# chymaera96/GraFP

Hardware: AMD Instinct MI355X
Metric: clips/sec contrastive step @ batch 1024 (higher is better)
Workload: dtype bf16; 1 GPU; contrastive step at global batch 1024 (1024 pairs/GPU x 1 GPU, global negatives), 1 s clips @16 kHz, mel->kNN-graph->GNN->NT-Xent, fwd+bwd+Adam, random-init GraphEncoder-t (18.4M params); global_batch=1024, parallelism=dp1, k=3

## Files before the change

grafp_amd/csrc/knn_split.hip:

```cpp
#include "dma_ring.h"
#include "elemio.h"
#include "knngraph.h"
#include "tuning.h"

namespace grafp {

constexpr int KS_KC = 32;
constexpr int KS_PLANE = KS_KC * KNN_TR * 2;
constexpr int KS_STAGE = 4 * KS_PLANE;
constexpr int KS_LDS = 2 * KS_STAGE + 3 * KNN_TR * 4;
constexpr float KS_SHIFT = 9.765625e-4f;

template <typename T>
__global__ __launch_bounds__(256) void knn_normalize_split_kernel(const T *__restrict__ x, int64_t sb, int64_t sc,
                                                                  float *__restrict__ den_out, float *__restrict__ sq,
                                                                  unsigned short *__restrict__ xh,
                                                                  unsigned short *__restrict__ xl, int C, int N,
                                                                  int *__restrict__ counters) {
    const int n = blockIdx.x * 256 + threadIdx.x;
    const int b = blockIdx.y;
    if (blockIdx.x == 0 && b == 0 && threadIdx.x < 2) counters[threadIdx.x] = 0;
    if (n >= N) return;
    const T *xb = x + (size_t)b * sb + n;
    const size_t o = (size_t)b * C * N + n;
// ... 110 lines not shown
        const int blk = t / nch, ch = t - blk * nch;
        const unsigned short *s = src0 + (size_t)(ch * KS_KC) * N + (wave >= 2 ? 0 : blk * KNN_TR);
        const unsigned st = lds0 + (t & 1) * KS_STAGE + wave * KS_PLANE;
#pragma unroll
        for (int i = 0; i < 8; ++i) gm_dma16(s + (size_t)(4 * i) * N, st + i * 1024);
        if (ch == 0 && wave < 2)
            gm_dma4(sqb + blk * KNN_TR + wave * 64 + lane, lds0 + 2 * KS_STAGE + ((blk % 3) * KNN_TR + wave * 64) * 4);
    };

    int foff[4];
#pragma unroll
    for (int tt = 0; tt < 4; ++tt) foff[tt] = ks_frag_offset(tt, lane, half);
    const int qoff = ks_frag_offset(wave, lane, half);

    f32x16 acc[4], prev[4];
#pragma unroll
    for (int t = 0; t < 4; ++t)
#pragma unroll
        for (int r = 0; r < 16; ++r) { acc[t][r] = 0.0f; prev[t][r] = 0.0f; }
    KeyList<K + 1> best;
    best.init();

    auto insert = [&](const f32x16 (&a)[4], int e, int sq_base, unsigned lane_bits) {
        const int loc_c = (e >> 4) * 32 + ((e & 15) & 3) + 8 * ((e & 15) >> 2);
        const float d = __builtin_fmaf(-2.0f, a[e >> 4][e & 15], dq) + sSq[sq_base + loc_c + 4 * half];
        best.push((__float_as_uint(d) & key_mask) | lane_bits | (unsigned)loc_c);
    };

    dma_chunk(0);
    gm_wait_vm<0>();
    __syncthreads();
    for (int blk = 0; blk < nblk; ++blk) {
        const int sq_prev = ((blk + 2) % 3) * KNN_TR;
        const unsigned bits_prev = (unsigned)((blk - 1) * KNN_TR) | (unsigned)(4 * half);
        for (int ch = 0; ch < nch; ++ch) {
            const int t = blk * nch + ch;
            if (t + 1 < T) dma_chunk(t + 1);
            const unsigned char *st = smem + (t & 1) * KS_STAGE;
#pragma unroll
            for (int ks = 0; ks < 2; ++ks) {
                const gm_bf16x8 qh = ks_frag(st + 2 * KS_PLANE, qoff + ks * 16 * 256);
                const gm_bf16x8 ql = ks_frag(st + 3 * KS_PLANE, qoff + ks * 16 * 256);
#pragma unroll
                for (int tt = 0; tt < 4; ++tt) {
                    const gm_bf16x8 ah = ks_frag(st, foff[tt] + ks * 16 * 256);
                    const gm_bf16x8 al = ks_frag(st + KS_PLANE, foff[tt] + ks * 16 * 256);
                    acc[tt] = __builtin_amdgcn_mfma_f32_32x32x16_bf16(al, qh, acc[tt], 0, 0, 0);
                    acc[tt] = __builtin_amdgcn_mfma_f32_32x32x16_bf16(ah, ql, acc[tt], 0, 0, 0);
                    acc[tt] = __builtin_amdgcn_mfma_f32_32x32x16_bf16(ah, qh, acc[tt], 0, 0, 0);
                }
                if (ch == 0 && blk > 0) {
#pragma unroll
                    for (int e = 0; e < 32; ++e) insert(prev, ks * 32 + e, sq_prev, bits_prev);
                }
            }
            gm_wait_vm<0>();
            __syncthreads();
        }
#pragma unroll
        for (int tt = 0; tt < 4; ++tt) {
            prev[tt] = acc[tt];
#pragma unroll
            for (int r = 0; r < 16; ++r) acc[tt][r] = 0.0f;
        }
    }
    {
        const unsigned bits_last = (unsigned)((nblk - 1) * KNN_TR) | (unsigned)(4 * half);
#pragma unroll
        for (int e = 0; e < 64; ++e) insert(prev, e, ((nblk + 2) % 3) * KNN_TR, bits_last);
    }
    unsigned ok[K + 1], onext = (unsigned)__shfl_xor((int)best.next, 32);
#pragma unroll
    for (int t = 0; t <= K; ++t) ok[t] = (unsigned)__shfl_xor((int)best.k[t], 32);
#pragma unroll
    for (int t = 0; t <= K; ++t) best.push(ok[t]);
    best.next = onext < best.next ? onext : best.next;
    if (half == 0)
        ks_classify_store<K>(best, key_mask, margin2, false, (size_t)b * N + myq, idx, unc_count, unc_flag, extra);
}

constexpr int KR_NS = 4;
constexpr int KR_STAGE = 2 * KS_PLANE;
constexpr int KR_NT = 8;
constexpr int KR_LDS = KR_NS * KR_STAGE + KR_NT * KNN_TR * 8;
constexpr float KR_TINY = 1.8189894e-12f;

template <int VE>
__global__ __launch_bounds__(256) void knn_norms_kernel(const unsigned short *__restrict__ x, int64_t sb, int64_t sc,
                                                        float *__restrict__ den_out, float *__restrict__ sq,
                                                        float2 *__restrict__ cs, int B, int C, int N,
                                                        int *__restrict__ counters) {
    const int per = N / VE;
    const int64_t gid = (int64_t)blockIdx.x * 256 + threadIdx.x;
    if (gid < 2) counters[gid] = 0;
    if (gid >= (int64_t)B * per) return;
    const int b = (int)(gid / per), n0 = (int)(gid - (int64_t)b * per) * VE;
    const unsigned short *xb = x + (size_t)b * sb + n0;
    float ss[VE], den[VE], q[VE];
#pragma unroll
    for (int u = 0; u < VE; ++u) ss[u] = 0.0f;
    auto load = [&](int c, unsigned (&w)[VE / 2]) {
        if (VE == 8) {
            const uint4 t = *reinterpret_cast<const uint4 *>(xb + (size_t)c * sc);
            w[0] = t.x; w[1 % (VE / 2)] = t.y; w[2 % (VE / 2)] = t.z; w[3 % (VE / 2)] = t.w;
        } else if (VE == 4) {
            const uint2 t = *reinterpret_cast<const uint2 *>(xb + (size_t)c * sc);
            w[0] = t.x; w[1 % (VE / 2)] = t.y;
        } else {
            w[0] = *reinterpret_cast<const unsigned *>(xb + (size_t)c * sc);
        }
    };
    for (int c = 0; c < C; c += 8) {
        unsigned w[8][VE / 2];
#pragma unroll
        for (int j = 0; j < 8; ++j) load(c + j, w[j]);
#pragma unroll
        for (int j = 0; j < 8; ++j)
#pragma unroll
            for (int e = 0; e < VE / 2; ++e) {
                const float lo = bf16_lo(w[j][e]), hi = bf16_hi(w[j][e]);
                ss[2 * e] = __builtin_fmaf(lo, lo, ss[2 * e]);
                ss[2 * e + 1] = __builtin_fmaf(hi, hi, ss[2 * e + 1]);
            }
    }
#pragma unroll
    for (int u = 0; u < VE; ++u) {
        den[u] = fmaxf(sqrtf(ss[u]), 1e-12f);
        q[u] = 0.0f;
    }
    for (int c = 0; c < C; c += 8) {
        unsigned w[8][VE / 2];
#pragma unroll
        for (int j = 0; j < 8; ++j) load(c + j, w[j]);
#pragma unroll
        for (int j = 0; j < 8; ++j)
#pragma unroll
            for (int e = 0; e < VE / 2; ++e) {
                const float lo = __fdiv_rn(bf16_lo(w[j][e]), den[2 * e]);
                const float hi = __fdiv_rn(bf16_hi(w[j][e]), den[2 * e + 1]);
                q[2 * e] = __builtin_fmaf(lo, lo, q[2 * e]);
                q[2 * e + 1] = __builtin_fmaf(hi, hi, q[2 * e + 1]);
            }
    }
    const size_t o = (size_t)b * N + n0;
#pragma unroll
    for (int u = 0; u < VE; ++u) {
        sq[o + u] = q[u];
        den_out[o + u] = den[u];
    }
    f32x4 *cs4 = reinterpret_cast<f32x4 *>(cs) + (o >> 1);
#pragma unroll
    for (int u = 0; u < VE; u += 2)
        cs4[u >> 1] = f32x4{-2.0f * __frcp_rn(den[u]), -2.0f * __frcp_rn(den[u + 1]), q[u], q[u + 1]};
}

template <int K, typename I>
__global__ __launch_bounds__(256, 2) void knn_topk_raw_kernel(const unsigned short *__restrict__ x, int64_t sb, int64_t sc,
                                                              const float *__restrict__ sq, const float *__restrict__ den,
                                                              const float2 *__restrict__ cs, I *__restrict__ idx,
                                                              int *__restrict__ unc_count,
                                                              unsigned char *__restrict__ unc_flag,
                                                              int *__restrict__ extra,
                                                              int C, int N, int tiles_per_clip, int nblocks,
                                                              float margin2, unsigned key_mask) {
    constexpr int D = KR_NS - 1;
    extern __shared__ __attribute__((aligned(16))) unsigned char smem[];
    const float2 *const sCS = reinterpret_cast<const float2 *>(smem + KR_NS * KR_STAGE);
    const unsigned lds0 = (unsigned)(uintptr_t)(gm_lptr)smem;

    const KnnCoords w = knn_coords(nblocks, tiles_per_clip);
    const int b = w.b, q0 = w.q0, lane = w.lane, half = w.half, l31 = w.l31;
    const int wave = __builtin_amdgcn_readfirstlane(w.wave);
    const int myq = q0 + wave * 32 + l31;
    const float iq = den[(size_t)b * N + myq];
    const float dqi = (sq[(size_t)b * N + myq] + KS_SHIFT) * iq;
    const float2 *csb = cs + (size_t)b * N;

    const int nch = C / KS_KC, nblk = N / KNN_TR, T = nblk * nch;

    const int pl = wave >> 1, hw = wave & 1;
    const int rowl = lane >> 4, sl = lane & 15;
    const int scol = (((sl >> 2) ^ (rowl & 3)) * 4 + (sl & 3)) * 8;
    const unsigned short *src0 = x + (size_t)b * sb + (size_t)(hw * 16 + rowl) * sc + scol + (pl ? q0 : 0);
    auto dma_chunk = [&](int t) {
        const int blk = t / nch, ch = t - blk * nch;
        const unsigned short *s = src0 + (size_t)(ch * KS_KC) * sc + (pl ? 0 : blk * KNN_TR);
        const unsigned st = lds0 + (t % KR_NS) * KR_STAGE + pl * KS_PLANE + hw * 4096;
#pragma unroll
        for (int i = 0; i < 4; ++i) gm_dma16(s + (size_t)(4 * i) * sc, st + i * 1024);
        if (ch == 0 && wave == 0)
            gm_dma16(csb + blk * KNN_TR + lane * 2, lds0 + KR_NS * KR_STAGE + (blk % KR_NT) * (KNN_TR * 8));
    };

    int foff[4];
#pragma unroll
    for (int tt = 0; tt < 4; ++tt) foff[tt] = ks_frag_offset(tt, lane, half);
    const int qoff = ks_frag_offset(wave, lane, half);

    f32x16 acc[4];
    KeyList<K + 1> best;
    best.init();
    bool bad = false;

    const gm_f32x2 iq2 = {iq, iq}, dqi2 = {dqi, dqi};
    unsigned kmv = key_mask;
    asm volatile("" : "+v"(kmv));
    auto insert4 = [&](const f32x16 (&a)[4], int e0, int tb, unsigned lane_bits) {
        const int tt = e0 >> 4, r0 = e0 & 15;
        const int loc_c = tt * 32 + 8 * (r0 >> 2);
        const f32x4 *tp = reinterpret_cast<const f32x4 *>(sCS + tb + loc_c + 4 * half);
        const f32x4 t01 = tp[0], t23 = tp[1];
        const gm_f32x2 d01 = __builtin_elementwise_fma(gm_f32x2{a[tt][r0], a[tt][r0 + 1]}, gm_f32x2{t01[0], t01[1]},
                                                    __builtin_elementwise_fma(gm_f32x2{t01[2], t01[3]}, iq2, dqi2));
        const gm_f32x2 d23 = __builtin_elementwise_fma(gm_f32x2{a[tt][r0 + 2], a[tt][r0 + 3]}, gm_f32x2{t23[0], t23[1]},
                                                    __builtin_elementwise_fma(gm_f32x2{t23[2], t23[3]}, iq2, dqi2));
        const unsigned c0 = lane_bits | (unsigned)loc_c;
        best.push((__float_as_uint(d01[0]) & kmv) | c0);
        best.push((__float_as_uint(d01[1]) & kmv) | (c0 + 1));
        best.push((__float_as_uint(d23[0]) & kmv) | (c0 + 2));
        best.push((__float_as_uint(d23[1]) & kmv) | (c0 + 3));
    };
    auto cj_of = [&](int tb, int c) -> float {
        return reinterpret_cast<const float *>(sCS + tb)[4 * (c >> 1) + (c & 1)];
    };

#pragma unroll
    for (int c = 0; c < D; ++c)
        if (c < T) dma_chunk(c);
    for (int blk = 0; blk < nblk; ++blk) {
        const int tb = (blk % KR_NT) * KNN_TR;
        const unsigned bits = (unsigned)(blk * KNN_TR);
        auto chunk = [&](int ch, auto first_c) __attribute__((always_inline)) {
            constexpr bool FIRST = decltype(first_c)::value;
            const int t = blk * nch + ch;
            {
                const int newer = T - 1 - t;
                if (newer >= D - 1) gm_wait_vm<(D - 1) * 4>();
                else if (newer == 1) gm_wait_vm<4>();
                else gm_wait_vm<0>();
                __builtin_amdgcn_s_barrier();
            }
            if (t + D < T) dma_chunk(t + D);
            const unsigned char *st = smem + (t % KR_NS) * KR_STAGE;
#pragma unroll
            for (int ks = 0; ks < 2; ++ks) {
                const gm_bf16x8 qf = ks_frag(st + KS_PLANE, qoff + ks * 16 * 256);
#pragma unroll
                for (int tt = 0; tt < 4; ++tt) {
                    const gm_bf16x8 af = ks_frag(st, foff[tt] + ks * 16 * 256);
                    if (FIRST && ks == 0) {
                        const f32x16 zero = {0.0f, 0.0f, 0.0f, 0.0f, 0.0f, 0.0f, 0.0f, 0.0f, 0.0f, 0.0f, 0.0f, 0.0f, 0.0f, 0.0f, 0.0f, 0.0f};
                        acc[tt] = __builtin_amdgcn_mfma_f32_32x32x16_bf16(af, qf, zero, 0, 0, 0);
                    } else {
                        acc[tt] = __builtin_amdgcn_mfma_f32_32x32x16_bf16(af, qf, acc[tt], 0, 0, 0);
                    }
                }
            }
        };
        chunk(0, KsBool<true>{});
        for (int ch = 1; ch < nch; ++ch) chunk(ch, KsBool<false>{});
#pragma unroll
        for (int e8 = 0; e8 < 64; e8 += 8) {
            insert4(acc, e8, tb, bits);
            insert4(acc, e8 + 4, tb, bits);
            __builtin_amdgcn_sched_barrier(0);
        }
        bad = bad || fabsf(cj_of(tb, lane)) < KR_TINY || fabsf(cj_of(tb, 64 + lane)) < KR_TINY;
    }
    const bool clip_bad = __any(bad ? 1 : 0) != 0;
#pragma unroll
    for (int t = 0; t <= K; ++t) best.k[t] |= (unsigned)(4 * half);
    best.next |= (unsigned)(4 * half);
    best.merge_halves();
    if (half == 0)
        ks_classify_store<K>(best, key_mask, margin2 * iq, clip_bad, (size_t)b * N + myq, idx, unc_count, unc_flag, extra);
}

template <int V> struct KsInt { static constexpr int value = V; };
constexpr int KX_QG = 16;
constexpr int KX_NU = 2;
constexpr int KX_CHUNK = 16384;

__host__ __device__ constexpr size_t kx_front_bytes(int K, int C) {
    const size_t heavy = (size_t)2 * KX_CHUNK + (size_t)KX_QG * C * 4, light = (size_t)4 * (K + 2) * C * 4;
    return heavy > light ? heavy : light;
}
template <int K, typename I, typename T>
__global__ __launch_bounds__(256) void knn_exact_clip_kernel(const T *__restrict__ x, int64_t sb, int64_t sc,
                                                             const float *__restrict__ den, const float *__restrict__ sq,
                                                             const unsigned char *__restrict__ unc_flag,
                                                             I *__restrict__ idx, int C, int N, int chc,
                                                             const int *__restrict__ counters,
                                                             int *__restrict__ n_uncertified,
                                                             const int *__restrict__ extra, int stop) {
    extern __shared__ __attribute__((aligned(16))) unsigned char sm_x[];
    if (n_uncertified && blockIdx.x == 0 && threadIdx.x == 0) *n_uncertified = counters[0];
    T *sX = reinterpret_cast<T *>(sm_x);
    float *sQ = reinterpret_cast<float *>(sm_x + 2 * KX_CHUNK);
    int *s_list = reinterpret_cast<int *>(sm_x + kx_front_bytes(K, C));
    __shared__ int s_n;
    __shared__ unsigned long long s_red[4];
    const int b = blockIdx.x, tid = threadIdx.x, lane = tid & 63;
    const int wave = __builtin_amdgcn_readfirstlane(tid >> 6);
    __shared__ int s_nl;
    if (tid == 0) { s_n = 0; s_nl = 0; }
    __syncthreads();
// ... 154 lines not shown
                    for (int s2 = 1; s2 < 64; s2 <<= 1) {
                        const unsigned long long other = __shfl_xor(m, s2);
                        m = other < m ? other : m;
                    }
                    if (lane == 0) s_red[wave] = m;
                    __syncthreads();
                    m = s_red[0];
#pragma unroll
                    for (int w = 1; w < 4; ++w) m = s_red[w] < m ? s_red[w] : m;
                    __syncthreads();
                    if (tid == 0) o[t] = (I)(unsigned)(m & 0xffffffffull);
                    if (mine == m) {
#pragma unroll
                        for (int u = 0; u + 1 < K; ++u) { mb.d[u] = mb.d[u + 1]; mb.i[u] = mb.i[u + 1]; }
                        mb.d[K - 1] = INFINITY;
                        mb.i[K - 1] = 0x7fffffff;
                    }
                }
            }
        }
    }
    };
    if (n <= 4) passes(KsInt<4>{});
    else passes(KsInt<KX_QG>{});
}

static int ks_index_bits(int N) {
    int b = 1;
    while ((1 << b) < N) ++b;
    return b;
}
static float ks_margin(int C) {
    const float e_g = 1.15e-5f + 3.6e-7f * (float)C;
    return 2.0f * e_g + 1.1920929e-7f * (float)C + 1e-6f;
}
static float ks_margin_raw(int C) { return 2.0f * (1.7881393e-7f * (float)C + 3.6e-7f) + 2e-6f; }
static bool ks_supported(int C, int N, int k) {
    return C > 0 && C % KS_KC == 0 && N >= KNN_TR && N % KNN_TR == 0 && N <= 4096 && k >= 1 && k <= 4 && k <= N &&
           ks_margin(C) < 0.9f * KS_SHIFT && kx_front_bytes(k, C) + (size_t)N * 4 <= 160 * 1024;
}

struct KsWs {
    float *sq, *den;
    unsigned short *xh, *xl;
    float2 *cs;
    int *count, *extra;
    unsigned char *flag;
};
static size_t ks_layout(void *ws, int dtype, int B, int C, int N, KsWs &p) {
    const size_t nodes = (size_t)B * N, e = nodes * C;
    WsCarve w{(char *)ws, 0};
    p.sq = w.take<float>(nodes * 4);
    p.den = w.take<float>(nodes * 4);
    p.xh = p.xl = nullptr;
    p.cs = nullptr;
    if (dtype == GRAFP_BF16) {
        p.cs = w.take<float2>(nodes * 8);
    } else {
        p.xh = w.take<unsigned short>(e * 2);
        p.xl = w.take<unsigned short>(e * 2);
    }
    p.count = w.take<int>(256);
    p.flag = w.take<unsigned char>(nodes);
    p.extra = w.take<int>(nodes * 4);
    return w.off;
}
static size_t ks_workspace(int dtype, int B, int C, int N) {
    KsWs p;
    return (B <= 0 || C <= 0 || N <= 0) ? 0 : ks_layout(nullptr, dtype, B, C, N, p);
}

struct KsArgs : KsWs {
    const void *x;
    bool f32, raw;
    int64_t sb, sc;
    int *n_unc;
    void *idx;
    int B, C, N;
    float margin2;
    unsigned key_mask;
};
template <int K, typename I, typename T> static void ks_launch_exact(const KsArgs &a, hipStream_t s) {
    const int wcols = a.N < 256 * KX_NU ? a.N : 256 * KX_NU;
    int chc = 32;
    while (chc > 1 && (size_t)chc * wcols * sizeof(T) > KX_CHUNK) chc >>= 1;
    const size_t lds_x = kx_front_bytes(K, a.C) + (size_t)a.N * 4;
    (void)hipFuncSetAttribute((const void *)knn_exact_clip_kernel<K, I, T>, hipFuncAttributeMaxDynamicSharedMemorySize,
                              (int)lds_x);
    hipLaunchKernelGGL((knn_exact_clip_kernel<K, I, T>), dim3(a.B), dim3(256), lds_x, s, (const T *)a.x, a.sb, a.sc, a.den,
                       a.sq, a.flag, (I *)a.idx, a.C, a.N, chc, a.count, a.n_unc, a.extra, GRAFP_TUNE_INT("GRAFP_KX_STOP", 0));
}
template <int K, typename I> static void ks_launch(const KsArgs &a, hipStream_t s) {
    const int tiles = a.N / KNN_TQ, nblocks = a.B * tiles;
    if (a.raw) {
        (void)hipFuncSetAttribute((const void *)knn_topk_raw_kernel<K, I>, hipFuncAttributeMaxDynamicSharedMemorySize, KR_LDS);
        hipLaunchKernelGGL((knn_topk_raw_kernel<K, I>), dim3(nblocks), dim3(256), KR_LDS, s, (const unsigned short *)a.x,
                           a.sb, a.sc, a.sq, a.den, a.cs, (I *)a.idx, a.count, a.flag, a.extra, a.C, a.N, tiles,
                           nblocks, a.margin2, a.key_mask);
    } else {
        (void)hipFuncSetAttribute((const void *)knn_topk_split_kernel<K, I>, hipFuncAttributeMaxDynamicSharedMemorySize, KS_LDS);
        hipLaunchKernelGGL((knn_topk_split_kernel<K, I>), dim3(nblocks), dim3(256), KS_LDS, s, a.xh, a.xl, a.sq, (I *)a.idx,
                           a.count, a.flag, a.extra, a.C, a.N, tiles, nblocks, a.margin2, a.key_mask);
    }
    if (a.f32) ks_launch_exact<K, I, float>(a, s);
    else ks_launch_exact<K, I, unsigned short>(a, s);
}
template <typename I> static void ks_launch_k(int k, const KsArgs &a, hipStream_t s) {
    switch (k) {
    case 1: ks_launch<1, I>(a, s); break;
    case 2: ks_launch<2, I>(a, s); break;
    case 3: ks_launch<3, I>(a, s); break;
    default: ks_launch<4, I>(a, s); break;
    }
}

}

extern "C" int grafp_knn_split_supported(int C, int N, int k) { return grafp::ks_supported(C, N, k) ? 1 : 0; }

extern "C" int grafp_knn_split_preferred(int C, int N, int k) { return grafp::ks_supported(C, N, k) && C <= 128 ? 1 : 0; }

extern "C" int grafp_knn_split_preferred_for(int dtype, int C, int N, int k) {
    if (dtype != GRAFP_BF16) return grafp_knn_split_preferred(C, N, k);
    return grafp::ks_supported(C, N, k) && C <= GRAFP_TUNE_INT("GRAFP_KNN_RAW_MAXC", 256) ? 1 : 0;
}

extern "C" size_t grafp_knn_split_workspace(int B, int C, int N) { return grafp::ks_workspace(GRAFP_F32, B, C, N); }
extern "C" size_t grafp_knn_split_workspace_for(int dtype, int B, int C, int N) {
    return grafp::ks_workspace(dtype, B, C, N);
}

extern "C" int grafp_knn_graph_split(const void *x, int dtype, int64_t stride_b, int64_t stride_c, int B, int C, int N,
                                     int k, void *idx, int idx_is_i32, void *ws, size_t ws_bytes, int32_t *n_uncertified,
                                     grafp_stream_t stream) {
    using namespace grafp;
    GRAFP_REQUIRE(x && idx, "knn_graph_split: null pointer");
    GRAFP_REQUIRE(B > 0 && ks_supported(C, N, k),
                  "knn_graph_split: unsupported shape B=%d C=%d N=%d k=%d (C %% 32, N %% 128, N <= 4096, k <= 4)", B, C, N, k);
    GRAFP_REQUIRE(dtype == GRAFP_F32 || dtype == GRAFP_BF16, "knn_graph_split: dtype %d not in {f32, bf16}", dtype);
    GRAFP_REQUIRE((int64_t)B * N < (1ll << 31), "knn_graph_split: too many nodes");
    KsArgs a;
    const size_t need = ks_layout(ws, dtype, B, C, N, a);
    if (!ws || ws_bytes < need) {
        set_error("knn_graph_split: workspace %zu bytes < required %zu", ws_bytes, need);
        return GRAFP_ERR_WORKSPACE;
    }
    hipStream_t s = (hipStream_t)stream;
    const bool raw = dtype == GRAFP_BF16;
    GRAFP_REQUIRE((((uintptr_t)ws | (uintptr_t)x) & 15) == 0 && (stride_b * (dtype == GRAFP_F32 ? 4 : 2)) % 16 == 0 &&
                      (stride_c * (dtype == GRAFP_F32 ? 4 : 2)) % 16 == 0,
                  "knn_graph_split: input rows and workspace must be 16-byte aligned");
    if (raw) {
        const int64_t nodes = (int64_t)B * N;
        const int ve = nodes >= (1 << 21) ? 8 : nodes >= (1 << 20) ? 4 : 2;
        const int64_t threads = nodes / ve;
        const dim3 gn((unsigned)((threads + 255) / 256));
        if (ve == 8)
            hipLaunchKernelGGL(knn_norms_kernel<8>, gn, dim3(256), 0, s, (const unsigned short *)x, stride_b, stride_c, a.den,
                               a.sq, a.cs, B, C, N, a.count);
        else if (ve == 4)
            hipLaunchKernelGGL(knn_norms_kernel<4>, gn, dim3(256), 0, s, (const unsigned short *)x, stride_b, stride_c, a.den,
                               a.sq, a.cs, B, C, N, a.count);
        else
            hipLaunchKernelGGL(knn_norms_kernel<2>, gn, dim3(256), 0, s, (const unsigned short *)x, stride_b, stride_c, a.den,
                               a.sq, a.cs, B, C, N, a.count);
        GRAFP_CHECK_LAUNCH("knn_norms_kernel");
    } else {
        const dim3 gn((N + 255) / 256, B);
        hipLaunchKernelGGL(knn_normalize_split_kernel<float>, gn, dim3(256), 0, s, (const float *)x, stride_b, stride_c,
                           a.den, a.sq, a.xh, a.xl, C, N, a.count);
        GRAFP_CHECK_LAUNCH("knn_normalize_split_kernel");
    }
    a.x = x; a.f32 = dtype == GRAFP_F32; a.raw = raw; a.sb = stride_b; a.sc = stride_c;
    a.n_unc = (int *)n_uncertified; a.idx = idx; a.B = B; a.C = C; a.N = N;
    a.margin2 = 2.0f * (raw ? ks_margin_raw(C) : ks_margin(C));
    a.key_mask = ~((1u << ks_index_bits(N)) - 1u);
    if (idx_is_i32) ks_launch_k<int32_t>(k, a, s);
    else ks_launch_k<int64_t>(k, a, s);
    GRAFP_CHECK_LAUNCH("knn_topk_split_kernel");
    return GRAFP_OK;
}
```

grafp_amd/csrc/mrconv.hip:

```cpp
#include <math.h>

#define GRAFP_STORE_FAMILY 3
#include "elemio.h"

namespace grafp {

constexpr int MR_THREADS = 256;

__device__ __forceinline__ int clampi(int64_t v, int n) {
    return v < 0 ? 0 : (v >= n ? n - 1 : (int)v);
}

template <typename T> constexpr int MR_NPAR = sizeof(T) == 4 ? 2 : 4;

__device__ __forceinline__ unsigned long long mr_fix_encode(float g, float scale) {
    const float v = __builtin_rintf(g * scale);
    const float hf = __builtin_truncf(v * 9.5367431640625e-7f);
    const float lf = __builtin_fmaf(hf, -1048576.0f, v);
    const int hi = (int)hf, lo = (int)lf;
    return ((unsigned long long)(unsigned)(hi + (lo >> 31)) << 32) | (unsigned long long)(unsigned)lo;
}
__device__ __forceinline__ float mr_fix_decode(unsigned long long a) {
    const int lo = (int)(unsigned)a;
    const int hi = (int)(unsigned)(a >> 32) - (lo >> 31);
// ... 220 lines not shown
                for (int e = 0; e < V; ++e) {
                    rows[c * N + n + e] = v[e];
                    acc[c * N + n + e] = 0;
                    base[c * N + n + e] = ge[e] - godd[it][e];
                    m = max(m, __float_as_uint(godd[it][e]) & 0x7fffffffu);
                }
            }
            MR_NEXT(V, N, c, n);
        }
    }
    mr_scale_publish(m, s_max, tid);
    stage_idx<I>(sidx, idx + (size_t)b * N * K, N, K, tid);
    __syncthreads();
    const MrScale fx = mr_scale_read(s_max);
    if (!fx.poisoned) {
        MR_WALK(V, tid, N, c, n);
#pragma unroll
        for (int it = 0; it < BWD_ITEMS; ++it) {
            if (c < cc) {
                const float *row = rows + c * N;
#pragma unroll
                for (int e = 0; e < V; ++e) {
                    const float xi = row[n + e];
                    float best = 0.0f;
                    int bj = 0;
                    for (int k = 0; k < K; ++k) {
                        const int j = sidx[k * N + n + e];
                        if (mr_first_max(k, row[j] - xi, best)) bj = j;
                    }
                    atomicAdd(reinterpret_cast<unsigned long long *>(&acc[c * N + bj]), fx.encode(godd[it][e]));
                }
            }
            MR_NEXT(V, N, c, n);
        }
    }
    __syncthreads();
    T *db = dx + (size_t)b * x_sb + (size_t)c0 * x_sc;
    MR_WALK(V, tid, N, c, n);
    while (c < cc) {
        if (V == 4) {
            float v[4];
#pragma unroll
            for (int e = 0; e < 4; ++e)
                v[e] = fx.out(base[c * N + n + e], (unsigned long long)acc[c * N + n + e]);
            ElemIO<T>::store(db + (size_t)c * x_sc + n, v, false);
        } else {
            ElemIO<T>::st1(db + (size_t)c * x_sc + n, fx.out(base[c * N + n], (unsigned long long)acc[c * N + n]));
        }
        MR_NEXT(V, N, c, n);
    }
}

constexpr int MRB_ITEMS = 2;
constexpr int MRB_SLAB = MRB_ITEMS * MR_THREADS * 4;

template <typename T, typename I>
__global__ __launch_bounds__(MR_THREADS) void mrconv_bwd_p_kernel(const T *__restrict__ x, int64_t x_sb, int64_t x_sc,
                                                                  const I *__restrict__ idx,
                                                                  const T *__restrict__ gout, int64_t g_sb,
                                                                  int64_t g_sc, T *__restrict__ dx, int C, int N, int K,
                                                                  int CC) {
    extern __shared__ __attribute__((aligned(16))) char smem[];
    __shared__ unsigned s_max[MR_THREADS / 64];
    const int b = blockIdx.y, tid = threadIdx.x;
    long long *acc = reinterpret_cast<long long *>(smem);
    float *rows = reinterpret_cast<float *>(acc + MRB_SLAB);
    int *sidx = reinterpret_cast<int *>(rows + MRB_SLAB);
    const int nslab = (C + CC - 1) / CC;
    const T *xb = x + (size_t)b * x_sb;
    const T *gb = gout + (size_t)b * g_sb;
    T *db = dx + (size_t)b * x_sb;
    int pc[MRB_ITEMS], pn[MRB_ITEMS];
    mr_pieces(tid, N, pc, pn);
    float pv[MRB_ITEMS][4], pe[MRB_ITEMS][4], po[MRB_ITEMS][4];
    auto fetch = [&](int slab) {
        const int c0 = slab * CC, cc = min(CC, C - c0);
#pragma unroll
        for (int it = 0; it < MRB_ITEMS; ++it)
            if (pc[it] < cc) {
                const int c = c0 + pc[it];
                ElemIO<T>::load(xb + (size_t)c * x_sc + pn[it], pv[it]);
                ElemIO<T>::load(gb + (size_t)(2 * c) * g_sc + pn[it], pe[it]);
                ElemIO<T>::load(gb + (size_t)(2 * c + 1) * g_sc + pn[it], po[it]);
            }
    };
    int slab = blockIdx.x;
    if (slab < nslab) fetch(slab);
    stage_idx<I>(sidx, idx + (size_t)b * N * K, N, K, tid);
    for (; slab < nslab; slab += gridDim.x) {
        const int c0 = slab * CC, cc = min(CC, C - c0);
        __syncthreads();
        float xi[MRB_ITEMS][4], godd[MRB_ITEMS][4], base[MRB_ITEMS][4];
        unsigned m = 0;
#pragma unroll
        for (int it = 0; it < MRB_ITEMS; ++it)
            if (pc[it] < cc) {
#pragma unroll
                for (int e = 0; e < 4; ++e) {
                    rows[pc[it] * N + pn[it] + e] = pv[it][e];
                    acc[pc[it] * N + pn[it] + e] = 0;
                    base[it][e] = pe[it][e] - po[it][e];
                    xi[it][e] = pv[it][e];
                    godd[it][e] = po[it][e];
                    m = max(m, __float_as_uint(po[it][e]) & 0x7fffffffu);
                }
            }
        mr_scale_publish(m, s_max, tid);
        __syncthreads();
        if (slab + gridDim.x < nslab) fetch(slab + gridDim.x);
        const MrScale fx = mr_scale_read(s_max);
#pragma unroll
        for (int it = 0; it < MRB_ITEMS; ++it) {
            if (pc[it] < cc) {
                const float *row = rows + pc[it] * N;
                float best[4] = {-INFINITY, -INFINITY, -INFINITY, -INFINITY};
                int bj[4];
                for (int k = 0; k < K; ++k) {
                    const int4 j4 = *reinterpret_cast<const int4 *>(sidx + k * N + pn[it]);
                    const int jj[4] = {j4.x, j4.y, j4.z, j4.w};
#pragma unroll
                    for (int e = 0; e < 4; ++e)
                        if (mr_first_max(k, row[jj[e]] - xi[it][e], best[e])) bj[e] = jj[e];
                }
                if (!fx.poisoned) {
#pragma unroll
                    for (int e = 0; e < 4; ++e)
                        atomicAdd(reinterpret_cast<unsigned long long *>(&acc[pc[it] * N + bj[e]]), fx.encode(godd[it][e]));
                }
            }
        }
        __syncthreads();
#pragma unroll
        for (int it = 0; it < MRB_ITEMS; ++it)
            if (pc[it] < cc) {
                float v[4];
#pragma unroll
                for (int e = 0; e < 4; ++e)
                    v[e] = fx.out(base[it][e], (unsigned long long)acc[pc[it] * N + pn[it] + e]);
                ElemIO<T>::store(db + (size_t)(c0 + pc[it]) * x_sc + pn[it], v, false);
            }
    }
}

template <typename T, typename I>
__global__ __launch_bounds__(MR_THREADS) void mrconv_bwd_a_kernel(const unsigned char *__restrict__ arg,
                                                                  const I *__restrict__ idx,
                                                                  const T *__restrict__ gout, int64_t g_sb,
                                                                  int64_t g_sc, T *__restrict__ dx, int64_t d_sb,
                                                                  int64_t d_sc, int C, int N, int K, int CC, int plain) {
    extern __shared__ __attribute__((aligned(16))) char smem[];
    __shared__ unsigned s_max[MR_THREADS / 64];
    const int b = blockIdx.y, tid = threadIdx.x;
    unsigned long long *acc = reinterpret_cast<unsigned long long *>(smem);
    int *sidx = reinterpret_cast<int *>(acc + MRB_SLAB);
    const int nslab = (C + CC - 1) / CC;
    int off[MRB_ITEMS], pn[MRB_ITEMS], pc[MRB_ITEMS];
    mr_pieces(tid, N, pc, pn);
#pragma unroll
    for (int it = 0; it < MRB_ITEMS; ++it) off[it] = pc[it] * N + pn[it];
    const T *ge_p[MRB_ITEMS];
    T *dx_p[MRB_ITEMS];
    const unsigned char *ar_p[MRB_ITEMS];
    const int64_t cstep = (int64_t)gridDim.x * CC;
#pragma unroll
    for (int it = 0; it < MRB_ITEMS; ++it) {
        const int64_t c = (int64_t)blockIdx.x * CC + pc[it];
        ge_p[it] = gout + (size_t)b * g_sb + (size_t)(2 * c) * g_sc + pn[it];
        dx_p[it] = dx + (size_t)b * d_sb + (size_t)c * d_sc + pn[it];
        ar_p[it] = arg + ((size_t)b * C + c) * (N / 4) + pn[it] / 4;
    }
    const int64_t ge_step = 2 * cstep * g_sc, dx_step = cstep * d_sc, ar_step = cstep * (N / 4);
    typedef typename ElemIO<T>::Raw4 Raw;
    constexpr int NPAR = MR_NPAR<T>;
    Raw pe[NPAR][MRB_ITEMS], po[NPAR][MRB_ITEMS];
    unsigned pa[NPAR][MRB_ITEMS];
    auto fetch = [&](int par, int slab) {
        const int cc = min(CC, C - slab * CC);
#pragma unroll
        for (int it = 0; it < MRB_ITEMS; ++it) {
            if (pc[it] < cc) {
                pe[par][it] = GRAFP_LD_ONCE(16, reinterpret_cast<const Raw *>(ge_p[it]));
                po[par][it] = GRAFP_LD_ONCE(16, reinterpret_cast<const Raw *>(ge_p[it] + g_sc));
                pa[par][it] = *ar_p[it];
            }
            ge_p[it] += ge_step;
            ar_p[it] += ar_step;
        }
    };
    int slab = blockIdx.x;
    const int G = gridDim.x;
#pragma unroll
    for (int par = 0; par < NPAR; ++par)
        if (slab + par * G < nslab) fetch(par, slab + par * G);
    stage_idx<I>(sidx, idx + (size_t)b * N * K, N, K, tid);
    while (slab < nslab) {
#pragma unroll
        for (int par = 0; par < NPAR; ++par) {
            if (slab < nslab) {
                const int cc = min(CC, C - slab * CC);
                __syncthreads();
                float godd[MRB_ITEMS][4], base[MRB_ITEMS][4];
                unsigned ak[MRB_ITEMS];
                unsigned m = 0;
#pragma unroll
                for (int it = 0; it < MRB_ITEMS; ++it)
                    if (pc[it] < cc) {
                        ak[it] = pa[par][it];
                        *reinterpret_cast<uint4 *>(acc + off[it]) = make_uint4(0, 0, 0, 0);
                        *reinterpret_cast<uint4 *>(acc + off[it] + 2) = make_uint4(0, 0, 0, 0);
                        float ge[4];
                        ElemIO<T>::unpack(pe[par][it], ge);
                        ElemIO<T>::unpack(po[par][it], godd[it]);
#pragma unroll
                        for (int e = 0; e < 4; ++e) {
                            base[it][e] = ge[e] - godd[it][e];
                            m = max(m, __float_as_uint(godd[it][e]) & 0x7fffffffu);
                        }
                    }
                mr_scale_publish(m, s_max, tid);
                __syncthreads();
                if (slab + NPAR * G < nslab) fetch(par, slab + NPAR * G);
                const MrScale fx = mr_scale_read(s_max);
                if (!fx.poisoned) {
#pragma unroll
                    for (int it = 0; it < MRB_ITEMS; ++it)
                        if (pc[it] < cc) {
                            unsigned long long *arow = acc + (off[it] - pn[it]);
                            int bj[4] = {0, 0, 0, 0};
                            for (int k = 0; k < K; ++k) {
                                const int4 j4 = *reinterpret_cast<const int4 *>(sidx + k * N + pn[it]);
                                const int jj[4] = {j4.x, j4.y, j4.z, j4.w};
#pragma unroll
                                for (int e = 0; e < 4; ++e) bj[e] = ((ak[it] >> (2 * e)) & 3u) == (unsigned)k ? jj[e] : bj[e];
                            }
#pragma unroll
                            for (int e = 0; e < 4; ++e) atomicAdd(arow + bj[e], fx.encode(godd[it][e]));
                        }
                }
                __syncthreads();
#pragma unroll
                for (int it = 0; it < MRB_ITEMS; ++it) {
                    if (pc[it] < cc) {
                        float v[4];
                        const uint4 a01 = *reinterpret_cast<const uint4 *>(acc + off[it]);
                        const uint4 a23 = *reinterpret_cast<const uint4 *>(acc + off[it] + 2);
                        const unsigned long long a[4] = {((unsigned long long)a01.y << 32) | a01.x,
                                                         ((unsigned long long)a01.w << 32) | a01.z,
                                                         ((unsigned long long)a23.y << 32) | a23.x,
                                                         ((unsigned long long)a23.w << 32) | a23.z};
#pragma unroll
                        for (int e = 0; e < 4; ++e) v[e] = fx.out(base[it][e], a[e]);
                        ElemIO<T>::store(dx_p[it], v, plain != 0);
                    }
                    dx_p[it] += dx_step;
                }
                slab += G;
            }
        }
    }
}

enum { MR_PATH_PERSISTENT = 0, MR_PATH_VEC4 = 1, MR_PATH_SCALAR = 2, MR_PATH_RECORD = 3 };
struct MrLaunch {
    int path;
    int items;
    int cc;
    int nslab, per_clip;
    size_t lds;
};
constexpr size_t MR_LDS_LIMIT = 160 * 1024;
constexpr int MR_FWD_ELEMS = 4096;
static_assert(MRB_SLAB <= MRP_SLAB, "a row that fits the backward slab fits the forward one");

static inline int mr_clamp_cc(int cc, int C) { return cc < 1 ? 1 : (cc > C ? C : cc); }

static int mr_choose(int64_t x_sb, int64_t x_sc, int64_t o_sb, int64_t o_sc, int N, int K, int C, int B,
                     bool aligned, bool backward, bool with_arg, MrLaunch *L) {
    const bool v4 = aligned && N % 4 == 0 && x_sb % 4 == 0 && x_sc % 4 == 0 && o_sb % 4 == 0 && o_sc % 4 == 0;
    const size_t edges = (size_t)K * N;
    const size_t lds_fwd_p = (MRP_SLAB + edges) * 4, lds_bwd_p = (3 * (size_t)MRB_SLAB + edges) * 4,
                 lds_bwd_a = (2 * (size_t)MRB_SLAB + edges) * 4;
    auto lds_generic = [&](int cc) {
        const size_t slab = (size_t)cc * N;
        return (backward ? 4 * ((slab + 1) & ~(size_t)1) + edges : slab + edges) * 4;
    };
    const bool record = with_arg && v4 && K <= 4 && N <= MRB_SLAB && lds_fwd_p <= MR_LDS_LIMIT && lds_bwd_a <= MR_LDS_LIMIT;
    const int slab = backward ? MRB_SLAB : MRP_SLAB;
    const size_t lds_p = !backward ? lds_fwd_p : (record ? lds_bwd_a : lds_bwd_p);
    if (record || (v4 && N <= slab && lds_p <= MR_LDS_LIMIT)) {
        *L = {record ? MR_PATH_RECORD : MR_PATH_PERSISTENT, backward ? MRB_ITEMS : MRP_ITEMS, std::min(slab / N, C), 0, 0, lds_p};
        L->nslab = (C + L->cc - 1) / L->cc;
        L->per_clip = L->nslab < 4 ? L->nslab : 4;
        while ((int64_t)L->per_clip * B < 1024 && L->per_clip < L->nslab) ++L->per_clip;
        return GRAFP_OK;
    }
    int items = 0, cc = mr_clamp_cc(MR_FWD_ELEMS / N, C);
    if (backward) {
        const int per_item = MR_THREADS * (v4 ? 4 : 1);
        items = N <= 2 * per_item ? 2 : 8;
        cc = mr_clamp_cc(items * per_item / N, C);
        GRAFP_REQUIRE((size_t)cc * N <= (size_t)items * per_item, "mrconv_bwd: N=%d exceeds the %d nodes a workgroup covers", N,
                      items * per_item);
        while (cc > 1 && lds_generic(cc) > MR_LDS_LIMIT) --cc;
    }
    GRAFP_REQUIRE(lds_generic(cc) <= MR_LDS_LIMIT, "mrconv_%s: N=%d K=%d needs %zu B of LDS (> 160 KiB)",
                  backward ? "bwd" : "fwd", N, K, lds_generic(cc));
    *L = {v4 ? MR_PATH_VEC4 : MR_PATH_SCALAR, items, cc, (C + cc - 1) / cc, (C + cc - 1) / cc, lds_generic(cc)};
    return GRAFP_OK;
}

static int mr_check_args(const char *op, bool pointers, int dtype, int B, int C, int N, int K) {
    GRAFP_REQUIRE(pointers, "%s: null pointer", op);
    GRAFP_REQUIRE(B > 0 && C > 0 && N > 0 && K > 0, "%s: bad shape B=%d C=%d N=%d K=%d", op, B, C, N, K);
    GRAFP_REQUIRE(dtype == GRAFP_F32 || dtype == GRAFP_BF16, "%s: dtype %d not in {f32, bf16}", op, dtype);
    return GRAFP_OK;
}

static bool mr_aligned(int dtype, const void *a, const void *b, const void *c = nullptr) {
    return (((uintptr_t)a | (uintptr_t)b | (uintptr_t)c) % (dtype == GRAFP_F32 ? 16 : 8)) == 0;
}

template <typename Kern, typename... Args>
static int mr_launch(const char *name, Kern kern, const MrLaunch &L, int B, grafp_stream_t stream, Args... args) {
    (void)hipFuncSetAttribute((const void *)kern, hipFuncAttributeMaxDynamicSharedMemorySize, (int)L.lds);
    hipLaunchKernelGGL(kern, dim3(L.per_clip, B), dim3(MR_THREADS), L.lds, (hipStream_t)stream, args...);
    GRAFP_CHECK_LAUNCH(name);
    return GRAFP_OK;
}

}

static int mrconv_fwd_impl(const char *op, const void *x, int dtype, int64_t x_sb, int64_t x_sc, const void *idx, int idx32,
                           int B, int C, int N, int K, void *out, int64_t o_sb, int64_t o_sc, grafp_stream_t stream,
                           unsigned char *arg = nullptr) {
    using namespace grafp;
    if (int e = mr_check_args(op, x && idx && out, dtype, B, C, N, K)) return e;
    MrLaunch L;
    if (int e = mr_choose(x_sb, x_sc, o_sb, o_sc, N, K, C, B, mr_aligned(dtype, x, out), false, arg != nullptr, &L)) return e;
    GRAFP_REQUIRE(!arg || L.path == MR_PATH_RECORD,
                  "mrconv_fwd_arg: shape / alignment outside grafp_mrconv_arg_supported (N=%d K=%d)", N, K);
    int rc = GRAFP_OK;
    for_elem_idx(dtype, idx32, [&](auto te, auto ti) {
        using T = typename decltype(te)::type;
        using I = typename decltype(ti)::type;
        if (L.path == MR_PATH_PERSISTENT || L.path == MR_PATH_RECORD) {
            const int plain = plain_stores((size_t)2 * B * C * N * sizeof(T), "GRAFP_MR_PLAIN_MAX_MB", 140);
            for_bool(arg != nullptr, [&](auto wk) {
                rc = mr_launch("mrconv_fwd_p_kernel", mrconv_fwd_p_kernel<T, I, decltype(wk)::value>, L, B, stream, (const T *)x,
                               x_sb, x_sc, (const I *)idx, (T *)out, o_sb, o_sc, C, N, K, L.cc, arg, plain);
            });
        } else {
            for_bool(L.path == MR_PATH_VEC4, [&](auto vec) {
                rc = mr_launch("mrconv_fwd_kernel", mrconv_fwd_kernel<T, decltype(vec)::value ? 4 : 1, I>, L, B, stream,
                               (const T *)x, x_sb, x_sc, (const I *)idx, (T *)out, o_sb, o_sc, C, N, K, L.cc);
            });
        }
    });
    return rc;
}

static int mrconv_bwd_impl(const char *op, const void *x, const unsigned char *arg, int dtype, int64_t x_sb, int64_t x_sc,
                           const void *idx, int idx32, const void *grad_out, int64_t g_sb, int64_t g_sc, int B, int C, int N,
                           int K, void *dx, grafp_stream_t stream) {
    using namespace grafp;
    if (int e = mr_check_args(op, (x || arg) && idx && grad_out && dx, dtype, B, C, N, K)) return e;
    MrLaunch L;
    if (int e = mr_choose(x_sb, x_sc, g_sb, g_sc, N, K, C, B, mr_aligned(dtype, x, grad_out, dx), true, arg != nullptr, &L)) return e;
    GRAFP_REQUIRE(!arg || L.path == MR_PATH_RECORD,
                  "mrconv_bwd_arg: shape / alignment outside grafp_mrconv_arg_supported (N=%d K=%d)", N, K);
    int rc = GRAFP_OK;
    for_elem_idx(dtype, idx32, [&](auto te, auto ti) {
        using T = typename decltype(te)::type;
        using I = typename decltype(ti)::type;
        if (L.path == MR_PATH_RECORD) {
            const int plain = plain_stores((size_t)B * C * N * sizeof(T), "GRAFP_MR_PLAIN_MAX_MB", 140);
            rc = mr_launch("mrconv_bwd_a_kernel", mrconv_bwd_a_kernel<T, I>, L, B, stream, arg, (const I *)idx,
                           (const T *)grad_out, g_sb, g_sc, (T *)dx, x_sb, x_sc, C, N, K, L.cc, plain);
        } else if (L.path == MR_PATH_PERSISTENT) {
            rc = mr_launch("mrconv_bwd_p_kernel", mrconv_bwd_p_kernel<T, I>, L, B, stream, (const T *)x, x_sb, x_sc,
                           (const I *)idx, (const T *)grad_out, g_sb, g_sc, (T *)dx, C, N, K, L.cc);
        } else {
            for_bool(L.path == MR_PATH_VEC4, [&](auto vec) {
                for_bool(L.items == 2, [&](auto two) {
                    rc = mr_launch("mrconv_bwd_kernel",
                                   mrconv_bwd_kernel<T, decltype(vec)::value ? 4 : 1, I, decltype(two)::value ? 2 : 8>, L, B,
                                   stream, (const T *)x, x_sb, x_sc, (const I *)idx, (const T *)grad_out, g_sb, g_sc, (T *)dx,
                                   C, N, K, L.cc);
                });
            });
        }
    });
    return rc;
}

extern "C" int grafp_mrconv_fwd_strided(const void *x, int dtype, int64_t x_sb, int64_t x_sc, const int64_t *idx, int B,
                                        int C, int N, int K, void *out, int64_t o_sb, int64_t o_sc,
                                        grafp_stream_t stream) {
    return mrconv_fwd_impl("mrconv_fwd", x, dtype, x_sb, x_sc, idx, 0, B, C, N, K, out, o_sb, o_sc, stream);
// ... 59 lines not shown
```

Measured before the change: 11190 clips/s.

## Add register-held kNN norms kernel and compact mrconv backward edge indexing

Adds a kNN norms kernel that keeps a node's whole bf16 feature column in registers, so the second normalization pass no longer reloads from memory. It is selected by default when C is small, and the per-thread vector width is reduced to keep register use bounded. Separately, the mrconv backward kernel stores the edge list as clamped 16-bit node-major indices and looks up each neighbor directly instead of looping over K with selects. It also zeroes the LDS accumulator after reading it rather than before each slab, which drops one barrier per slab. The barrier removal relies on the existing later syncs to order the zeroing against the next slab's atomics, and 16-bit indices assume N fits in 16 bits.

```diff
diff --git a/grafp_amd/csrc/knn_split.hip b/grafp_amd/csrc/knn_split.hip
--- a/grafp_amd/csrc/knn_split.hip
+++ b/grafp_amd/csrc/knn_split.hip
@@ -286,6 +286,125 @@
 #pragma unroll
     for (int u = 0; u < VE; u += 2)
         cs4[u >> 1] = f32x4{-2.0f * __frcp_rn(den[u]), -2.0f * __frcp_rn(den[u + 1]), q[u], q[u + 1]};
+}
+
+constexpr int KN_HELD = 128;
+template <int VE>
+__global__ __launch_bounds__(256, VE == 8 ? 2 : 3) void knn_norms_held_kernel(const unsigned short *__restrict__ x, int64_t sb, int64_t sc,
+                                                                float *__restrict__ den_out, float *__restrict__ sq,
+                                                                float2 *__restrict__ cs, int B, int C, int N,
+                                                                int *__restrict__ counters) {
+    constexpr int GW = 4 * VE;
+    constexpr int NG = KN_HELD / GW;
+    const int per = N / VE;
+    const int64_t gid = (int64_t)blockIdx.x * 256 + threadIdx.x;
+    if (gid < 2) counters[gid] = 0;
+    if (gid >= (int64_t)B * per) return;
+    const int b = (int)(gid / per), n0 = (int)(gid - (int64_t)b * per) * VE;
+    const unsigned short *xb = x + (size_t)b * sb + n0;
+    unsigned w[NG][GW];
+#pragma unroll
+    for (int g = 0; g < NG; ++g) {
+        if (8 * g < C) {
+            const unsigned short *p = xb + (size_t)(8 * g) * sc;
+#pragma unroll
+            for (int j = 0; j < 8; ++j) {
+                if constexpr (VE == 8) {
+                    const uint4 t = *reinterpret_cast<const uint4 *>(p + (size_t)j * sc);
+                    w[g][4 * j] = t.x; w[g][4 * j + 1] = t.y; w[g][4 * j + 2] = t.z; w[g][4 * j + 3] = t.w;
+                } else if constexpr (VE == 4) {
+                    const uint2 t = *reinterpret_cast<const uint2 *>(p + (size_t)j * sc);
+                    w[g][2 * j] = t.x; w[g][2 * j + 1] = t.y;
+                } else if constexpr (VE == 2) {
+                    w[g][j] = *reinterpret_cast<const unsigned *>(p + (size_t)j * sc);
+                } else if ((j & 1) == 0) {
+                    w[g][j >> 1] = *reinterpret_cast<const unsigned *>(p + (size_t)(j + (n0 & 1)) * sc - (n0 & 1));
+                }
+            }
+        }
+    }
+    if constexpr (VE == 1) {
+        const unsigned sel = (n0 & 1) ? 0x03020706u : 0x05040100u;
+#pragma unroll
+        for (int g = 0; g < NG; ++g)
+            if (8 * g < C)
+#pragma unroll
+                for (int i = 0; i < GW; ++i) {
+                    const unsigned other = (unsigned)__builtin_amdgcn_update_dpp(0, (int)w[g][i], 0xB1, 0xf, 0xf, false);
+                    w[g][i] = __builtin_amdgcn_perm(other, w[g][i], sel);
+                }
+    }
+    auto each = [&](int g, auto &&f) __attribute__((always_inline)) {
+#pragma unroll
+        for (int j = 0; j < 8; ++j) {
+            if constexpr (VE == 1) {
+                const unsigned d = w[g][j >> 1];
+                f(0, (j & 1) ? bf16_hi(d) : bf16_lo(d));
+            } else {
+#pragma unroll
+                for (int e = 0; e < VE / 2; ++e) {
+                    const unsigned d = w[g][j * (VE / 2) + e];
+                    f(2 * e, bf16_lo(d));
+                    f(2 * e + 1, bf16_hi(d));
+                }
+            }
+            if ((j + 1) * VE % 8 == 0) __builtin_amdgcn_sched_barrier(0);
+        }
+    };
+    float ss[VE], den[VE], q[VE];
+#pragma unroll
+    for (int u = 0; u < VE; ++u) ss[u] = 0.0f;
+#pragma unroll
+    for (int g = 0; g < NG; ++g)
+        if (8 * g < C) {
+            each(g, [&](int u, float v) { ss[u] = __builtin_fmaf(v, v, ss[u]); });
+        }
+#pragma unroll
+    for (int u = 0; u < VE; ++u) {
+        den[u] = fmaxf(sqrtf(ss[u]), 1e-12f);
+        q[u] = 0.0f;
+    }
+#pragma unroll
+    for (int g = 0; g < NG; ++g)
+#pragma unroll
+        for (int i = 0; i < GW; ++i) asm volatile("" : "+v"(w[g][i]));
+#pragma unroll
+    for (int g = 0; g < NG; ++g)
+        if (8 * g < C) {
+            each(g, [&](int u, float v) {
+                const float t = __fdiv_rn(v, den[u]);
+                q[u] = __builtin_fmaf(t, t, q[u]);
+            });
+        }
+    const size_t o = (size_t)b * N + n0;
+#pragma unroll
+    for (int u = 0; u < VE; ++u) {
+        sq[o + u] = q[u];
+        den_out[o + u] = den[u];
+    }
+    if constexpr (VE == 1) {
+        float *t = reinterpret_cast<float *>(cs) + 4 * (o >> 1) + (o & 1);
+        t[0] = -2.0f * __frcp_rn(den[0]);
+        t[2] = q[0];
+    } else {
+        f32x4 *cs4 = reinterpret_cast<f32x4 *>(cs) + (o >> 1);
+#pragma unroll
+        for (int u = 0; u < VE; u += 2)
+            cs4[u >> 1] = f32x4{-2.0f * __frcp_rn(den[u]), -2.0f * __frcp_rn(den[u + 1]), q[u], q[u + 1]};
+    }
+}
+
+struct KnPlan {
+    int ve;
+    bool held;
+};
+static KnPlan kn_plan(int64_t nodes, int C) {
+    KnPlan p = {nodes >= (1 << 21) ? 8 : nodes >= (1 << 20) ? 4 : 2, false};
+    if (C <= 2 * KN_HELD && GRAFP_TUNE_INT("GRAFP_KNN_NORMS_HELD", 1)) {
+        p.held = true;
+        while (p.ve > 1 && p.ve * C > 2 * KN_HELD) p.ve >>= 1;
+    }
+    return p;
 }
 
 template <int K, typename I>
@@ -746,18 +865,22 @@
                   "knn_graph_split: input rows and workspace must be 16-byte aligned");
     if (raw) {
         const int64_t nodes = (int64_t)B * N;
-        const int ve = nodes >= (1 << 21) ? 8 : nodes >= (1 << 20) ? 4 : 2;
-        const int64_t threads = nodes / ve;
-        const dim3 gn((unsigned)((threads + 255) / 256));
-        if (ve == 8)
-            hipLaunchKernelGGL(knn_norms_kernel<8>, gn, dim3(256), 0, s, (const unsigned short *)x, stride_b, stride_c, a.den,
-                               a.sq, a.cs, B, C, N, a.count);
-        else if (ve == 4)
-            hipLaunchKernelGGL(knn_norms_kernel<4>, gn, dim3(256), 0, s, (const unsigned short *)x, stride_b, stride_c, a.den,
-                               a.sq, a.cs, B, C, N, a.count);
-        else
-            hipLaunchKernelGGL(knn_norms_kernel<2>, gn, dim3(256), 0, s, (const unsigned short *)x, stride_b, stride_c, a.den,
-                               a.sq, a.cs, B, C, N, a.count);
+        const KnPlan np = kn_plan(nodes, C);
+        const dim3 gn((unsigned)((nodes / np.ve + 255) / 256));
+        auto norms = [&](auto kern) {
+            hipLaunchKernelGGL(kern, gn, dim3(256), 0, s, (const unsigned short *)x, stride_b, stride_c, a.den, a.sq, a.cs, B, C,
+                               N, a.count);
+        };
+        if (np.held) {
+            if (np.ve == 8) norms(knn_norms_held_kernel<8>);
+            else if (np.ve == 4) norms(knn_norms_held_kernel<4>);
+            else if (np.ve == 2) norms(knn_norms_held_kernel<2>);
+            else norms(knn_norms_held_kernel<1>);
+        } else {
+            if (np.ve == 8) norms(knn_norms_kernel<8>);
+            else if (np.ve == 4) norms(knn_norms_kernel<4>);
+            else norms(knn_norms_kernel<2>);
+        }
         GRAFP_CHECK_LAUNCH("knn_norms_kernel");
     } else {
         const dim3 gn((N + 255) / 256, B);
diff --git a/grafp_amd/csrc/mrconv.hip b/grafp_amd/csrc/mrconv.hip
--- a/grafp_amd/csrc/mrconv.hip
+++ b/grafp_amd/csrc/mrconv.hip
@@ -396,7 +396,7 @@
     __shared__ unsigned s_max[MR_THREADS / 64];
     const int b = blockIdx.y, tid = threadIdx.x;
     unsigned long long *acc = reinterpret_cast<unsigned long long *>(smem);
-    int *sidx = reinterpret_cast<int *>(acc + MRB_SLAB);
+    unsigned short *sedge = reinterpret_cast<unsigned short *>(acc + MRB_SLAB);
     const int nslab = (C + CC - 1) / CC;
     int off[MRB_ITEMS], pn[MRB_ITEMS], pc[MRB_ITEMS];
     mr_pieces(tid, N, pc, pn);
@@ -436,13 +436,20 @@
 #pragma unroll
     for (int par = 0; par < NPAR; ++par)
         if (slab + par * G < nslab) fetch(par, slab + par * G);
-    stage_idx<I>(sidx, idx + (size_t)b * N * K, N, K, tid);
+    {
+        const I *idxb = idx + (size_t)b * N * K;
+        for (int i = tid; i < N * K; i += MR_THREADS) sedge[i] = (unsigned short)clampi((int64_t)idxb[i], N);
+    }
+#pragma unroll
+    for (int it = 0; it < MRB_ITEMS; ++it) {
+        *reinterpret_cast<uint4 *>(acc + off[it]) = make_uint4(0, 0, 0, 0);
+        *reinterpret_cast<uint4 *>(acc + off[it] + 2) = make_uint4(0, 0, 0, 0);
+    }
     while (slab < nslab) {
 #pragma unroll
         for (int par = 0; par < NPAR; ++par) {
             if (slab < nslab) {
                 const int cc = min(CC, C - slab * CC);
-                __syncthreads();
                 float godd[MRB_ITEMS][4], base[MRB_ITEMS][4];
                 unsigned ak[MRB_ITEMS];
                 unsigned m = 0;
@@ -450,8 +457,6 @@
                 for (int it = 0; it < MRB_ITEMS; ++it)
                     if (pc[it] < cc) {
                         ak[it] = pa[par][it];
-                        *reinterpret_cast<uint4 *>(acc + off[it]) = make_uint4(0, 0, 0, 0);
-                        *reinterpret_cast<uint4 *>(acc + off[it] + 2) = make_uint4(0, 0, 0, 0);
                         float ge[4];
                         ElemIO<T>::unpack(pe[par][it], ge);
                         ElemIO<T>::unpack(po[par][it], godd[it]);
@@ -470,13 +475,10 @@
                     for (int it = 0; it < MRB_ITEMS; ++it)
                         if (pc[it] < cc) {
                             unsigned long long *arow = acc + (off[it] - pn[it]);
-                            int bj[4] = {0, 0, 0, 0};
-                            for (int k = 0; k < K; ++k) {
-                                const int4 j4 = *reinterpret_cast<const int4 *>(sidx + k * N + pn[it]);
-                                const int jj[4] = {j4.x, j4.y, j4.z, j4.w};
-#pragma unroll
-                                for (int e = 0; e < 4; ++e) bj[e] = ((ak[it] >> (2 * e)) & 3u) == (unsigned)k ? jj[e] : bj[e];
-                            }
+                            const unsigned short *erow = sedge + pn[it] * K;
+                            int bj[4];
+#pragma unroll
+                            for (int e = 0; e < 4; ++e) bj[e] = erow[e * K + min((int)((ak[it] >> (2 * e)) & 3u), K - 1)];
 #pragma unroll
                             for (int e = 0; e < 4; ++e) atomicAdd(arow + bj[e], fx.encode(godd[it][e]));
                         }
@@ -488,6 +490,8 @@
                         float v[4];
                         const uint4 a01 = *reinterpret_cast<const uint4 *>(acc + off[it]);
                         const uint4 a23 = *reinterpret_cast<const uint4 *>(acc + off[it] + 2);
+                        *reinterpret_cast<uint4 *>(acc + off[it]) = make_uint4(0, 0, 0, 0);
+                        *reinterpret_cast<uint4 *>(acc + off[it] + 2) = make_uint4(0, 0, 0, 0);
                         const unsigned long long a[4] = {((unsigned long long)a01.y << 32) | a01.x,
                                                          ((unsigned long long)a01.w << 32) | a01.z,
                                                          ((unsigned long long)a23.y << 32) | a23.x,
```

Result: no change. 11260 clips/s, median of 6 (+0.7%).
